# andywag/streaming_data_loader

Hardware: AMD Instinct MI355X
Metric: device-resident tokenize+mask MB/s of input text, seq_len=512, 1/2/4/8 MI355X (higher is better)
Workload: dtype u8->int32

## Files before the change

### streaming_data_loader_amd/csrc/kernels.hpp

```cpp
#pragma once

#include <hip/hip_runtime.h>

#include <cstdint>

#include "common.hpp"
#include "zstd_format.hpp"

namespace sdl {

hipError_t launch_chunk_ranges(const uint64_t *off, int64_t R, int64_t N, uint32_t *ranges, hipStream_t st,
                               uint32_t *rb1 = nullptr, uint32_t *zero1 = nullptr, const void *copy_src = nullptr,
                               void *copy_dst = nullptr, size_t copy_bytes = 0);

hipError_t launch_wordpiece_chunks(const DevTok &T, const DevFirst &F, bool cased, const uint8_t *text, int64_t N,
                                   const uint64_t *off, int64_t R,
                                   uint32_t *ranges, uint16_t *tokc, uint32_t *chunk_cnt, uint32_t *rec_local,
                                   hipStream_t st, int64_t c_begin = 0, int64_t c_end = -1);

struct BpeLong {
    uint64_t pos;
    uint32_t len;
    uint32_t chunk;
    uint32_t k;
// ... 87 lines not shown
    const uint64_t *nominal;
    const uint64_t *found;
    uint32_t n_chunks;
    const uint32_t *tgt0;
    uint16_t *slots;
    uint32_t cap;
    uint64_t *end_bit;
    uint64_t *end_hdr;
    uint32_t *next;
    uint32_t *len;
    uint32_t *flags;
    int32_t *status;
    const uint64_t *mend;
};
hipError_t launch_gz_find(const uint8_t *in, uint64_t ma, uint64_t mz, const uint64_t *nominal, uint64_t n_chunks,
                          uint64_t span, uint64_t *found, uint32_t *stats, hipStream_t st);
hipError_t launch_inflate_chunks(const uint8_t *in, const GzChunkArgs &a, uint64_t n_list, hipStream_t st);
inline uint64_t gz_window_group(uint64_t n) {
    uint64_t g = 1;
    while (g * g < n) ++g;
    return g;
}
hipError_t launch_gz_windows(const uint16_t *slots, uint32_t cap, const uint32_t *order, const uint32_t *len,
                             uint64_t n_order, uint8_t *windows, uint16_t *gmaps, uint8_t *gwin, hipStream_t st);
hipError_t launch_gz_resolve(const uint16_t *slots, uint32_t cap, const uint32_t *order, const uint32_t *len,
                             const uint64_t *pos, uint64_t n_order, const uint8_t *windows, uint8_t *out,
                             uint32_t *crc, uint32_t *shift, const X2N &x2n, int32_t *status, hipStream_t st);
hipError_t launch_gz_crc_fold(const uint32_t *crc, const uint32_t *shift, uint64_t n_order, const uint8_t *trailer,
                              const int32_t *status, int32_t *mstatus, hipStream_t st);

int64_t scan_tmp_words(int64_t n);
hipError_t launch_exclusive_scan(const uint32_t *in, uint32_t *out, int64_t n, uint32_t *tmp, hipStream_t st,
                                 const uint32_t *carry_in = nullptr);

enum : int32_t {
    ZS_OK = zs::OK,
    ZS_E_RANGE = zs::E_RANGE,
    ZS_E_TRUNC = zs::E_TRUNC,
    ZS_E_MAGIC = zs::E_MAGIC,
    ZS_E_DICT = zs::E_DICT,
    ZS_E_WINDOW = zs::E_WINDOW,
    ZS_E_BTYPE = zs::E_BTYPE,
    ZS_E_BSIZE = zs::E_BSIZE,
    ZS_E_LITHDR = zs::E_LITHDR,
    ZS_E_HUF = zs::E_HUF,
    ZS_E_FSE = zs::E_FSE,
    ZS_E_SEQHDR = zs::E_SEQHDR,
    ZS_E_ENDBITS = zs::E_ENDBITS,
    ZS_E_FAR = zs::E_FAR,
    ZS_E_SIZE = zs::E_SIZE,
    ZS_E_CHECKSUM = zs::E_CHECKSUM,
    ZS_E_STALL = zs::E_STALL
};
hipError_t launch_zs_index(const uint8_t *zst, uint64_t len, const uint64_t *foff, uint64_t n, zs::Frame *frames,
                           zs::Block *blocks, const uint32_t *first_block, uint32_t *nblk, uint32_t block_cap,
                           hipStream_t st);
hipError_t launch_zs_parse(const uint8_t *zst, const zs::Frame *frames, zs::Block *blocks, uint32_t nb, hipStream_t st);
hipError_t launch_zs_link(zs::Frame *frames, zs::Block *blocks, uint64_t n, uint32_t *lit_tot, uint32_t *seq_tot,
                          unsigned long long *totals, hipStream_t st);
hipError_t launch_zs_decode(const uint8_t *zst, const zs::Frame *frames, zs::Block *blocks, uint32_t nb,
                            const uint32_t *lit_base, const uint32_t *seq_base, uint8_t *lit, zs::SeqRec *seq,
                            hipStream_t st);
hipError_t launch_zs_chain(zs::Frame *frames, zs::Block *blocks, uint64_t n, uint32_t *out_size,
                           unsigned long long *totals, hipStream_t st);
hipError_t launch_zs_write(const uint8_t *zst, zs::Frame *frames, const zs::Block *blocks, uint32_t nb, uint64_t n,
                           const uint32_t *lit_base, const uint32_t *seq_base, const uint8_t *lit, const zs::SeqRec *seq,
                           const uint32_t *ooff, uint8_t *out, bool check, int32_t *status, uint32_t *bad,
                           hipStream_t st, hipEvent_t *ev = nullptr);

constexpr int MAX_SEGMENTS = 16;
struct SegChunks {
    int64_t cb[MAX_SEGMENTS + 1];
    int K;
};
hipError_t launch_seg_bounds(const uint32_t *ranges, const SegChunks &sc, int64_t R, uint32_t *rb, hipStream_t st);
hipError_t launch_scan_range(const uint32_t *in, uint32_t *out, const uint32_t *rb, int k, hipStream_t st);

hipError_t launch_compact_tokens(const uint32_t *tokc, const uint32_t *chunk_cnt, const uint32_t *chunk_off,
                                 int64_t n_chunks, uint32_t *tok, const uint32_t *long_count,
                                 const uint32_t *chunk_ent, const BpeLong *long_list, const uint16_t *long_scratch,
                                 hipStream_t st, const uint32_t *long_pool = nullptr, int64_t stride = STAGE,
                                 bool list16 = false);


struct SegSel {
    const uint32_t *rb;
    int k;
    int last;
};

hipError_t launch_records(const RowParams &P, const uint64_t *off, int64_t R, int64_t N, const uint32_t *chunk_off,
                          int64_t n_chunks, const uint32_t *rec_local, uint32_t *rec_tok, uint32_t *rec_cnt,
                          uint32_t *rec_rows, SegSel sel, hipStream_t st);

struct DirectDst {
    int32_t *ids[2], *am[2], *tt[2], *lab[2];
    uint32_t base, cap, B, pad;
};
struct RowOut {
    int32_t *input_ids, *attention_mask, *token_type_ids, *labels;
    float *labels_f32;
    DirectDst direct;
};

constexpr int64_t SMALL_CHUNKS = 64;
struct SmallDown {
    const uint32_t *tokc, *chunk_cnt;
    uint32_t *chunk_off, *tok;
    const uint32_t *long_count, *chunk_ent;
    const BpeLong *long_list;
    const uint16_t *long_scratch;
    const uint32_t *long_pool;
    int64_t stride;
    int list16;
    const uint32_t *rec_local;
    uint32_t *rec_tok, *rec_cnt, *rec_rows, *row_off, *row_rec;
    uint32_t *stat;
    const uint32_t *tok_err;
    int rows;
    RowOut out;
};
hipError_t launch_downstream_small(const SmallDown &d, const RowParams &P, const uint64_t *off, int64_t R, int64_t N,
                                   hipStream_t st);

struct TokSrc {
    const uint32_t *tok;
    const uint16_t *lists;
    const uint32_t *chunk_off;
    int64_t n_lists;
    const uint32_t *row_chunk;
};

struct RowChunkIn {
    uint32_t *row_chunk;
    const uint32_t *rec_tok, *rec_cnt, *chunk_off;
    const uint64_t *off;
    int64_t n_lists;
    int32_t S, n_pre, chunk;
};
hipError_t launch_row_map(const uint32_t *row_off, int64_t R, uint32_t *row_rec, SegSel sel, hipStream_t st,
                          const RowChunkIn *rc = nullptr);

struct RowSeg {
    int32_t *ids, *am, *tt, *lab;
    uint32_t g0, n, dst, pad;
};
hipError_t launch_rows_to_host(const RowSeg *segs, int n_segs, uint32_t rows_per_seg_max, const int32_t *ids,
                               const int32_t *am, const int32_t *tt, const int32_t *lab, int S, int LW,
                               hipStream_t st);

hipError_t launch_rows_direct(const DirectDst &d, const uint32_t *row_off, int64_t R, const int32_t *ids,
                              const int32_t *am, const int32_t *tt, const int32_t *lab, int S, int LW,
                              const uint32_t *err0, const uint32_t *err1, uint32_t *stat, hipStream_t st);

struct MaskPolicy {
    int32_t policy;
    int32_t per_mille;
    uint32_t vocab_size;
    uint32_t pad;
    const uint32_t *cont_bits;
};

hipError_t launch_rows(const RowParams &P, const TokSrc &src, const uint32_t *rec_tok, const uint32_t *rec_cnt,
                       const uint32_t *row_off, const uint32_t *row_rec, SegSel sel, int64_t rows_cap, RowOut out,
                       hipStream_t st,
                       hipStream_t st_late = nullptr, const MaskPolicy *mp = nullptr);
struct PackParams {
    const uint32_t *tok, *rec_tok, *rec_cnt;
    uint32_t *rec_len;
    uint32_t *pk_off;
    int64_t R, rows_cap;
    int32_t S, B, eos, min_ids;
    const int32_t *carry_ids, *carry_pos;
    const uint32_t *carry_len;
// ... 59 lines not shown
```

### streaming_data_loader_amd/csrc/pipeline.hip

```cpp
#include "common.hpp"
#include "device_util.hpp"
#include "kernels.hpp"
#include "rows_device.hpp"

namespace sdl {

constexpr int SCAN_NT = 256;
constexpr int SCAN_PER = 8;
constexpr int SCAN_TILE = SCAN_NT * SCAN_PER;

__global__ __launch_bounds__(SCAN_NT) void k_scan_reduce(const uint32_t *__restrict__ in, int64_t n,
                                                         uint32_t *__restrict__ sums) {
    __shared__ uint32_t scratch[SCAN_NT / 64];
    const int64_t base = (int64_t)blockIdx.x * SCAN_TILE + (int64_t)threadIdx.x * SCAN_PER;
    uint32_t s = 0;
#pragma unroll
    for (int k = 0; k < SCAN_PER; ++k)
        if (base + k < n) s += in[base + k];
    uint32_t tot;
    block_excl_sum<SCAN_NT>(s, &tot, scratch);
    if (threadIdx.x == 0) sums[blockIdx.x] = tot;
}

__global__ __launch_bounds__(SCAN_NT) void k_scan_sums(uint32_t *__restrict__ sums, int64_t nb,
                                                       const uint32_t *carry_in) {
    __shared__ uint32_t scratch[SCAN_NT / 64];
    uint32_t carry = carry_in ? *carry_in : 0u;
    for (int64_t t0 = 0; t0 < nb; t0 += SCAN_TILE) {
        const int64_t base = t0 + (int64_t)threadIdx.x * SCAN_PER;
        uint32_t v[SCAN_PER], s = 0;
#pragma unroll
        for (int k = 0; k < SCAN_PER; ++k) {
            v[k] = base + k < nb ? sums[base + k] : 0u;
            s += v[k];
        }
        uint32_t tot;
        uint32_t ex = block_excl_sum<SCAN_NT>(s, &tot, scratch) + carry;
#pragma unroll
        for (int k = 0; k < SCAN_PER; ++k) {
            if (base + k < nb) sums[base + k] = ex;
            ex += v[k];
        }
        carry += tot;
    }
    if (threadIdx.x == 0) sums[nb] = carry;
}

__global__ __launch_bounds__(SCAN_NT) void k_scan_apply(const uint32_t *__restrict__ in, int64_t n,
                                                        const uint32_t *__restrict__ sums, int64_t nb,
                                                        uint32_t *__restrict__ out) {
    __shared__ uint32_t scratch[SCAN_NT / 64];
    const int64_t base = (int64_t)blockIdx.x * SCAN_TILE + (int64_t)threadIdx.x * SCAN_PER;
    uint32_t v[SCAN_PER], s = 0;
#pragma unroll
    for (int k = 0; k < SCAN_PER; ++k) {
        v[k] = base + k < n ? in[base + k] : 0u;
        s += v[k];
    }
    uint32_t tot;
    uint32_t ex = block_excl_sum<SCAN_NT>(s, &tot, scratch) + sums[blockIdx.x];
#pragma unroll
    for (int k = 0; k < SCAN_PER; ++k) {
        if (base + k < n) out[base + k] = ex;
        ex += v[k];
    }
    if (blockIdx.x == 0 && threadIdx.x == 0) out[n] = sums[nb];
}

constexpr int SCAN_SMALL_NT = 1024, SCAN_SMALL_PER = 8;
constexpr int64_t SCAN_SMALL = (int64_t)SCAN_SMALL_NT * SCAN_SMALL_PER;
__global__ __launch_bounds__(SCAN_SMALL_NT) void k_scan_small(const uint32_t *__restrict__ in, int64_t n,
                                                              uint32_t *__restrict__ out, const uint32_t *carry_in) {
    __shared__ uint32_t scratch[SCAN_SMALL_NT / 64];
    const uint32_t carry = carry_in ? *carry_in : 0u;
    __syncthreads();
    const int64_t base = (int64_t)threadIdx.x * SCAN_SMALL_PER;
    uint32_t v[SCAN_SMALL_PER], s = 0;
#pragma unroll
    for (int k = 0; k < SCAN_SMALL_PER; ++k) {
        v[k] = base + k < n ? in[base + k] : 0u;
        s += v[k];
    }
    uint32_t tot;
    uint32_t ex = block_excl_sum<SCAN_SMALL_NT>(s, &tot, scratch) + carry;
#pragma unroll
    for (int k = 0; k < SCAN_SMALL_PER; ++k) {
        if (base + k < n) out[base + k] = ex;
        ex += v[k];
    }
    if (threadIdx.x == 0) out[n] = carry + tot;
}

int64_t scan_tmp_words(int64_t n) { return (n + SCAN_TILE - 1) / SCAN_TILE + 1; }

hipError_t launch_exclusive_scan(const uint32_t *in, uint32_t *out, int64_t n, uint32_t *tmp, hipStream_t st,
                                 const uint32_t *carry_in) {
    if (n <= 0) return carry_in ? hipSuccess : hipMemsetAsync(out, 0, sizeof(uint32_t), st);
    if (n <= SCAN_SMALL) {
        hipLaunchKernelGGL(k_scan_small, dim3(1), dim3(SCAN_SMALL_NT), 0, st, in, n, out, carry_in);
        return hipGetLastError();
    }
    const int64_t nb = (n + SCAN_TILE - 1) / SCAN_TILE;
    hipLaunchKernelGGL(k_scan_reduce, dim3((unsigned)nb), dim3(SCAN_NT), 0, st, in, n, tmp);
    hipLaunchKernelGGL(k_scan_sums, dim3(1), dim3(SCAN_NT), 0, st, tmp, nb, carry_in);
    hipLaunchKernelGGL(k_scan_apply, dim3((unsigned)nb), dim3(SCAN_NT), 0, st, in, n, tmp, nb, out);
    return hipGetLastError();
}

__global__ void k_seg_bounds(const uint32_t *__restrict__ ranges, SegChunks sc, int64_t R, uint32_t *__restrict__ rb) {
    const int k = (int)threadIdx.x;
    if (k > sc.K) return;
    uint32_t v;
    if (k == 0) v = 0;
    else if (k == sc.K) v = (uint32_t)R;
    else {
        const uint32_t q = ranges[3 * sc.cb[k] + 2];
        v = q == 0 ? 0u : q - 1u;
        if (v > (uint32_t)R) v = (uint32_t)R;
    }
    rb[k] = v;
}

hipError_t launch_seg_bounds(const uint32_t *ranges, const SegChunks &sc, int64_t R, uint32_t *rb, hipStream_t st) {
    hipLaunchKernelGGL(k_seg_bounds, dim3(1), dim3(64), 0, st, ranges, sc, R, rb);
    return hipGetLastError();
}

constexpr int RSCAN_NT = 1024, RSCAN_PER = 8;
__global__ __launch_bounds__(RSCAN_NT) void k_scan_range(const uint32_t *__restrict__ in, uint32_t *__restrict__ out,
                                                         const uint32_t *__restrict__ rb, int k) {
    __shared__ uint32_t scratch[RSCAN_NT / 64];
    const int64_t a = rb[k], b = rb[k + 1];
    uint32_t carry = k > 0 ? out[a] : 0u;
    __syncthreads();
    for (int64_t t0 = a; t0 < b; t0 += (int64_t)RSCAN_NT * RSCAN_PER) {
        const int64_t base = t0 + (int64_t)threadIdx.x * RSCAN_PER;
        uint32_t v[RSCAN_PER], sum = 0;
#pragma unroll
        for (int j = 0; j < RSCAN_PER; ++j) {
            v[j] = base + j < b ? in[base + j] : 0u;
// ... 3 lines not shown
        uint32_t ex = block_excl_sum<RSCAN_NT>(sum, &tot, scratch) + carry;
#pragma unroll
        for (int j = 0; j < RSCAN_PER; ++j) {
            if (base + j < b) out[base + j] = ex;
            ex += v[j];
        }
        carry += tot;
    }
    if (threadIdx.x == 0) out[b] = carry;
}

hipError_t launch_scan_range(const uint32_t *in, uint32_t *out, const uint32_t *rb, int k, hipStream_t st) {
    hipLaunchKernelGGL(k_scan_range, dim3(1), dim3(RSCAN_NT), 0, st, in, out, rb, k);
    return hipGetLastError();
}

struct RowSpan {
    int64_t g_lo, g_real, g_end;
};
__device__ __forceinline__ RowSpan row_span(const SegSel &s, const uint32_t *row_off, int B, int64_t rows_cap) {
    const uint32_t r0 = s.rb[s.k], r1 = s.rb[s.k + 1];
    RowSpan x;
    x.g_lo = row_off[r0];
    x.g_real = row_off[r1];
    x.g_end = x.g_real;
    if (s.last) {
        int64_t Gpad = (x.g_real + B - 1) / B * B;
        if (Gpad > rows_cap) Gpad = rows_cap;
        x.g_end = Gpad > x.g_real ? Gpad : x.g_real;
    }
    return x;
}

__global__ __launch_bounds__(256) void k_chunk_ranges(const uint64_t *__restrict__ off, int64_t R, int64_t n_chunks,
                                                      uint32_t *__restrict__ ranges, uint32_t *__restrict__ rb1,
                                                      uint32_t *__restrict__ zero1, const uint4 *__restrict__ csrc,
                                                      uint4 *__restrict__ cdst, int64_t cn16) {
    const int64_t c = (int64_t)blockIdx.x * 256 + threadIdx.x;
    for (int64_t x = c; x < cn16; x += (int64_t)gridDim.x * 256) cdst[x] = csrc[x];
    if (c == 0) {
        if (rb1) {
            rb1[0] = 0u;
            rb1[1] = (uint32_t)R;
        }
        if (zero1) *zero1 = 0u;
    }
    if (c >= n_chunks) return;
    auto lower = [&](int64_t x) {
        int64_t lo = 0, hi = R + 1;
        while (lo < hi) {
            const int64_t m = (lo + hi) >> 1;
            if ((int64_t)off[m] < x) lo = m + 1; else hi = m;
        }
        return lo;
    };
    const int64_t c0 = c * CHUNK;
    ranges[3 * c + 0] = (uint32_t)lower(c0 - HALO_L);
    ranges[3 * c + 1] = (uint32_t)lower(c0 - HALO_L + WIN);
    ranges[3 * c + 2] = (uint32_t)lower(c0);
}

hipError_t launch_chunk_ranges(const uint64_t *off, int64_t R, int64_t N, uint32_t *ranges, hipStream_t st,
                               uint32_t *rb1, uint32_t *zero1, const void *copy_src, void *copy_dst, size_t copy_bytes) {
    const int64_t n_chunks = (N + CHUNK - 1) / CHUNK;
    const int64_t cn16 = copy_src ? (int64_t)((copy_bytes + 15) / 16) : 0;
    if (n_chunks == 0 && cn16 == 0) return hipSuccess;
    int64_t blocks = (n_chunks + 255) / 256;
    const int64_t cb = (cn16 + 255) / 256;
    if (cb > blocks) blocks = cb < 64 ? cb : 64;
    if (blocks < 1) blocks = 1;
    hipLaunchKernelGGL(k_chunk_ranges, dim3((unsigned)blocks), dim3(256), 0, st, off, R, n_chunks, ranges, rb1, zero1,
                       (const uint4 *)copy_src, (uint4 *)copy_dst, cn16);
    return hipGetLastError();
}

template <int PART, bool E16 = false>
__global__ __launch_bounds__(256) void k_compact_tokens(const uint32_t *__restrict__ tokc,
                                                        const uint32_t *__restrict__ chunk_cnt,
                                                        const uint32_t *__restrict__ chunk_off, int64_t n_chunks,
                                                        uint32_t *__restrict__ tok, const uint32_t *long_count,
                                                        const uint32_t *__restrict__ chunk_ent,
                                                        const BpeLong *__restrict__ long_list,
// ... 4 lines not shown
    compact_wave<PART, E16>(cb, tokc, chunk_cnt, chunk_off, n_chunks, tok, long_count, chunk_ent, long_list,
                            long_scratch, long_pool, stride);
}

hipError_t launch_compact_tokens(const uint32_t *tokc, const uint32_t *chunk_cnt, const uint32_t *chunk_off,
                                 int64_t n_chunks, uint32_t *tok, const uint32_t *long_count,
                                 const uint32_t *chunk_ent, const BpeLong *long_list, const uint16_t *long_scratch,
                                 hipStream_t st, const uint32_t *long_pool, int64_t stride, bool list16) {
    if (n_chunks == 0) return hipSuccess;
    const int64_t waves = (n_chunks + COMPACT_CPW - 1) / COMPACT_CPW;
    if (list16) {
        hipLaunchKernelGGL((k_compact_tokens<1, true>), dim3((unsigned)((waves + 3) / 4)), dim3(256), 0, st, tokc,
                           chunk_cnt, chunk_off, n_chunks, tok, nullptr, nullptr, nullptr, nullptr, nullptr, stride);
        return hipGetLastError();
    }
    hipLaunchKernelGGL(k_compact_tokens<1>, dim3((unsigned)((waves + 3) / 4)), dim3(256), 0, st, tokc, chunk_cnt,
                       chunk_off, n_chunks, tok, long_count, chunk_ent, long_list, long_scratch, long_pool, stride);
    if (long_count)
        hipLaunchKernelGGL(k_compact_tokens<2>, dim3((unsigned)((waves + 3) / 4)), dim3(256), 0, st, tokc, chunk_cnt,
                           chunk_off, n_chunks, tok, long_count, chunk_ent, long_list, long_scratch, long_pool, stride);
    return hipGetLastError();
}

__global__ __launch_bounds__(256) void k_records(RowParams P, const uint64_t *__restrict__ off, int64_t R, int64_t N,
                                                 const uint32_t *__restrict__ chunk_off, int64_t n_chunks,
                                                 const uint32_t *__restrict__ rec_local, uint32_t *__restrict__ rec_tok,
                                                 uint32_t *__restrict__ rec_cnt, uint32_t *__restrict__ rec_rows,
                                                 SegSel sel) {
    const int64_t r_lo = sel.rb[sel.k], r_hi = sel.rb[sel.k + 1];
    for (int64_t r = r_lo + (int64_t)blockIdx.x * 256 + threadIdx.x; r < r_hi; r += (int64_t)gridDim.x * 256)
        record_one(P, off, r, N, chunk_off, n_chunks, rec_local, rec_tok, rec_cnt, rec_rows);
}

hipError_t launch_records(const RowParams &P, const uint64_t *off, int64_t R, int64_t N, const uint32_t *chunk_off,
                          int64_t n_chunks, const uint32_t *rec_local, uint32_t *rec_tok, uint32_t *rec_cnt,
                          uint32_t *rec_rows, SegSel sel, hipStream_t st) {
    if (R == 0) return hipSuccess;
    const int64_t want = (R + 255) / 256;
    hipLaunchKernelGGL(k_records, dim3((unsigned)(want < 1024 ? want : 1024)), dim3(256), 0, st, P, off, R, N,
                       chunk_off, n_chunks, rec_local, rec_tok, rec_cnt, rec_rows, sel);
    return hipGetLastError();
}

template <bool RC>
__global__ __launch_bounds__(256) void k_row_map(const uint32_t *__restrict__ row_off, uint32_t *__restrict__ row_rec,
                                                 SegSel sel, RowChunkIn rc) {
    const int64_t r_lo = sel.rb[sel.k], r_hi = sel.rb[sel.k + 1];
    for (int64_t r = r_lo + (int64_t)blockIdx.x * 256 + threadIdx.x; r < r_hi; r += (int64_t)gridDim.x * 256) {
        const uint32_t g0 = row_off[r], g1 = row_off[r + 1];
        if constexpr (RC) {
            if (g0 == g1) continue;
            ListBracket br = list_bracket(rc.off[r], rc.off[r + 1], rc.n_lists);
            const uint32_t t0 = rc.rec_tok[r], cnt = rc.rec_cnt[r];
            for (uint32_t g = g0; g < g1; ++g) {
                row_rec[g] = (uint32_t)r;
                const int64_t base = rc.chunk ? (int64_t)(g - g0) * rc.S : 0;
                const int64_t rel0 = base > rc.n_pre ? base - rc.n_pre : 0;
                if (rel0 < (int64_t)cnt) br.lo = list_chunk_of(rc.chunk_off, br.lo, br.hi, t0 + (uint32_t)rel0);
                rc.row_chunk[g] = (uint32_t)br.lo;
            }
        } else {
            for (uint32_t g = g0; g < g1; ++g) row_rec[g] = (uint32_t)r;
        }
    }
}

__device__ __forceinline__ void block_scan_small(const uint32_t *__restrict__ in, int64_t n, uint32_t *__restrict__ out,
                                                 uint32_t *scratch) {
    const int64_t base = (int64_t)threadIdx.x * SCAN_SMALL_PER;
    uint32_t v[SCAN_SMALL_PER], s = 0;
#pragma unroll
    for (int k = 0; k < SCAN_SMALL_PER; ++k) {
        v[k] = base + k < n ? in[base + k] : 0u;
        s += v[k];
    }
    uint32_t tot;
    uint32_t ex = block_excl_sum<SCAN_SMALL_NT>(s, &tot, scratch);
#pragma unroll
    for (int k = 0; k < SCAN_SMALL_PER; ++k) {
        if (base + k < n) out[base + k] = ex;
        ex += v[k];
    }
    if (threadIdx.x == 0) out[n] = tot;
}

hipError_t launch_row_map(const uint32_t *row_off, int64_t R, uint32_t *row_rec, SegSel sel, hipStream_t st,
                          const RowChunkIn *rc) {
    if (R == 0) return hipSuccess;
    const int64_t want = (R + 255) / 256;
    const dim3 grid((unsigned)(want < 1024 ? want : 1024));
    if (rc) hipLaunchKernelGGL(k_row_map<true>, grid, dim3(256), 0, st, row_off, row_rec, sel, *rc);
    else hipLaunchKernelGGL(k_row_map<false>, grid, dim3(256), 0, st, row_off, row_rec, sel, RowChunkIn{});
    return hipGetLastError();
}

constexpr int ROWS_WAVES = 7;
constexpr int ROWS_WAVES4 = 1;
// ... 1301 lines not shown
```

### streaming_data_loader_amd/csrc/rows_device.hpp

```cpp
#pragma once
#include "common.hpp"
#include "device_util.hpp"
#include "kernels.hpp"
#include "list_index.hpp"
#include "mlm_pick.hpp"

namespace sdl {

static_assert(LIST_CHUNK == CHUNK && LIST_STRIDE == STAGE, "list_index.hpp restates the chunk geometry");

constexpr int COMPACT_CPW = 4;
template <int PART = 0, bool E16 = false>
__device__ __forceinline__ void compact_wave(int64_t cb, const uint32_t *__restrict__ tokc,
                                             const uint32_t *__restrict__ chunk_cnt,
                                             const uint32_t *__restrict__ chunk_off, int64_t n_chunks,
                                             uint32_t *__restrict__ tok, const uint32_t *long_count,
                                             const uint32_t *__restrict__ chunk_ent,
                                             const BpeLong *__restrict__ long_list,
                                             const uint16_t *__restrict__ long_scratch,
                                             const uint32_t *__restrict__ long_pool, int64_t stride) {
    const int lane = threadIdx.x & 63;
    uint32_t n[COMPACT_CPW], o[COMPACT_CPW];
#pragma unroll
    for (int j = 0; j < COMPACT_CPW; ++j) {
// ... 75 lines not shown
                    const uint16_t *jr = reinterpret_cast<const uint16_t *>(tokc + (cb + j) * stride + UNI_JR_OFF) +
                                         (x[j] & 0xFFFu);
                    for (uint32_t q0 = 0; q0 < w[j]; q0 += 8) {
                        uint32_t id[8];
#pragma unroll
                        for (uint32_t r = 0; r < 8; ++r) id[r] = q0 + r < w[j] ? jr[q0 + r] : 0u;
#pragma unroll
                        for (uint32_t r = 0; r < 8; ++r)
                            if (q0 + r < w[j]) dst[at + q0 + r] = id[r];
                    }
                } else if (long_pool) {
                    const uint32_t po = x[j] & 0x7FFFFFFFu;
                    for (uint32_t q = 0; q < w[j]; ++q) dst[at + q] = long_pool[po + 1 + q];
                } else {
                    const uint64_t pos = long_list[x[j] & 0x7FFFFFFFu].pos;
                    for (uint32_t q = 0; q < w[j]; ++q) dst[at + q] = long_scratch[pos + q];
                }
            }
            written[j] += (uint32_t)lane_bcast((int)incl, 63);
        }
    }
}

__device__ __forceinline__ void compact_small(const SmallDown &d, int64_t cb, const uint32_t *__restrict__ chunk_off,
                                              int64_t n_chunks) {
    if (d.list16)
        compact_wave<0, true>(cb, d.tokc, d.chunk_cnt, chunk_off, n_chunks, d.tok, nullptr, nullptr, nullptr, nullptr,
                              nullptr, d.stride);
    else
        compact_wave(cb, d.tokc, d.chunk_cnt, chunk_off, n_chunks, d.tok, d.long_count, d.chunk_ent, d.long_list,
                     d.long_scratch, d.long_pool, d.stride);
}

__device__ __forceinline__ void record_one(const RowParams &P, const uint64_t *__restrict__ off, int64_t r, int64_t N,
                                           const uint32_t *__restrict__ chunk_off, int64_t n_chunks,
                                           const uint32_t *__restrict__ rec_local, uint32_t *__restrict__ rec_tok,
                                           uint32_t *__restrict__ rec_cnt, uint32_t *__restrict__ rec_rows) {
    auto tok_off = [&](int64_t q) -> uint32_t {
        const int64_t p = (int64_t)off[q];
        return p >= N ? chunk_off[n_chunks] : chunk_off[p / CHUNK] + rec_local[q];
    };
    const uint32_t a = tok_off(r), b = tok_off(r + 1);
    const uint32_t cnt = b - a;
    const uint32_t n = cnt + (uint32_t)(P.n_pre + P.n_post);
    uint32_t rows = 0;
    if (n >= (uint32_t)P.min_ids) rows = P.chunk ? ceil_div_u32(n, (uint32_t)P.S) : 1u;
    rec_tok[r] = a;
    rec_cnt[r] = cnt;
    rec_rows[r] = rows;
}

__device__ __forceinline__ uint4 philox4x32_10(uint4 c, uint32_t k0, uint32_t k1) {
#pragma unroll
    for (int r = 0; r < 10; ++r) {
        const uint32_t lo0 = 0xD2511F53u * c.x, hi0 = __umulhi(0xD2511F53u, c.x);
        const uint32_t lo1 = 0xCD9E8D57u * c.z, hi1 = __umulhi(0xCD9E8D57u, c.z);
        c = make_uint4(hi1 ^ c.y ^ k0, lo1, hi0 ^ c.w ^ k1, lo0);
        k0 += 0x9E3779B9u;
        k1 += 0xBB67AE85u;
    }
    return c;
}

__device__ __forceinline__ uint32_t mlm_key(uint64_t seed, uint64_t rec, uint32_t chunk, uint32_t pos) {
    const uint4 c = philox4x32_10(make_uint4(pos >> 2, chunk, (uint32_t)rec, (uint32_t)(rec >> 32)), (uint32_t)seed,
                                  (uint32_t)(seed >> 32));
    const uint32_t s = pos & 3u;
    return s == 0 ? c.x : s == 1 ? c.y : s == 2 ? c.z : c.w;
}

__device__ __forceinline__ int32_t frame_id(const int32_t (&a)[MAX_FRAME], int k) {
    return k == 0 ? a[0] : k == 1 ? a[1] : k == 2 ? a[2] : a[3];
}

template <int MR>
__device__ __forceinline__ void select_k_smallest(const uint32_t (&key)[MR][4], int k, bool (&sel)[MR][4]) {
    if (k <= 0) {
#pragma unroll
        for (int m = 0; m < MR; ++m)
#pragma unroll
            for (int w = 0; w < 4; ++w) sel[m][w] = false;
        return;
// ... 595 lines not shown
```

### streaming_data_loader_amd/csrc/sdl_batcher.cpp

```cpp
#include <dlfcn.h>
#include <hip/hip_runtime.h>

#include <algorithm>
#include <chrono>
#include <cstdlib>
#include <cmath>
#include <cstdio>
#include <cstring>
#include <deque>
#include <memory>
#include <mutex>
#include <stdexcept>
#include <string>
#include <thread>
#include <vector>

#include "../../include/sdl_batcher.h"
#include "assets.hpp"
#include "kernels.hpp"
#include "pack_queue.hpp"

using namespace sdl;

namespace {
// ... 433 lines not shown
        HIP_TRY(launch_pack_flush(pack_params(0, rows_cap), st));
        pk_cur ^= 1;
        pk_ran = true;
        last_rows_cap = rows_cap;
        last_R = 0;
    }

    int64_t rows_capacity(int64_t N, int64_t R) const {
        const int64_t F = P.n_pre + P.n_post;
        const int64_t ids = dt.kind == TOK_UNIGRAM ? 2 * N + 1024 * 1024 : N;
        int64_t cap = P.chunk ? (ids + R * (F + P.S - 1)) / P.S + 1 : R;
        if (pack()) cap = (ids + R + P.S - 1) / P.S + 1;
        return (cap + P.B - 1) / P.B * P.B;
    }

    void run_device(const uint8_t *d_text, int64_t N, const uint64_t *d_off, int64_t R, uint64_t first_record,
                    hipStream_t st, const uint32_t *d_labels = nullptr, const uint64_t *d_label_off = nullptr) {
        const int64_t n_chunks = (N + CHUNK - 1) / CHUNK;
        const int64_t rows_cap = rows_capacity(N, R);
        if (pack() && rows_cap * P.S > ((int64_t)1 << 32) - 4096)
            throw CapacityError("pack: the call's rows exceed 2^32 positions");
        ranges.ensure((size_t)std::max<int64_t>(n_chunks, 1) * 3);
        const bool wp = dt.kind != TOK_BYTE_BPE && dt.kind != TOK_UNIGRAM;
        tokc.ensure((size_t)std::max<int64_t>(n_chunks, 1) * (dt.kind == TOK_UNIGRAM ? UNI_STAGE : wp ? STAGE / 2 : STAGE));
        chunk_cnt.ensure((size_t)n_chunks + 1);
        chunk_off.ensure((size_t)n_chunks + 1);
        rec_local.ensure((size_t)R + 1);
        const size_t tok_ids_n = dt.kind == TOK_UNIGRAM ? (size_t)2 * N + 1024 * 1024 + 1 : (size_t)N + 1;
        if (!wp || span()) tok_ids.ensure(tok_ids_n);
        rec_tok.ensure((size_t)R + 1);
        rec_cnt.ensure((size_t)R + 1);
        rec_rows.ensure((size_t)R + 1);
        row_off.ensure((size_t)R + 1);
        scan_tmp.ensure((size_t)std::max(scan_tmp_words(n_chunks), scan_tmp_words(R)) + 1);
        const size_t plane = (size_t)std::max<int64_t>(rows_cap, 1) * P.S;
        o_ids.ensure(plane);
        o_am.ensure(plane);
        if (plane4()) o_tt.ensure(plane);
        if (multi()) {
            o_f32.ensure((size_t)std::max<int64_t>(rows_cap, 1) * P.label_width);
            lab_err.ensure(1);
        } else {
            o_lab.ensure((size_t)std::max<int64_t>(rows_cap, 1) * P.label_width);
            if (single()) lab_err.ensure(1);
        }
        row_rec.ensure((size_t)std::max<int64_t>(rows_cap, 1));
        const bool rm1 = P.task == SDL_TASK_MLM && P.rng_mode == 1;
        const bool policy = P.task == SDL_TASK_MLM && mpol.policy != 0;
        const int mask_w = (P.S + 31) / 32;

        RowParams p = P;
        p.first_record = first_record;
        p.mask_w = mask_w;
        p.mask_bits0 = nullptr;
        p.mask_spos = nullptr;
        p.mask_off = d_off;
        p.mask_R = R;
        p.mask_spec1 = 0;
        const bool bpe = dt.kind == TOK_BYTE_BPE;
        const bool uni = dt.kind == TOK_UNIGRAM;
        SegChunks sc{};
        sc.K = 1;
        if (!bpe && !uni && seg_target > 1 && n_chunks >= 2 * seg_min_chunks) {
            sc.K = (int)std::min<int64_t>(seg_target, n_chunks / seg_min_chunks);
            sc.K = std::min(sc.K, MAX_SEGMENTS);
        }
        for (int k = 0; k <= sc.K; ++k) sc.cb[k] = n_chunks * k / sc.K;
// ... 45 lines not shown
            SmallDown d{tokc.p, chunk_cnt.p, chunk_off.p, tok_ids.p,
                        uni ? uni_counters.p : bpe ? long_count.p : nullptr,
                        uni || bpe ? chunk_ent.p : nullptr, bpe ? long_list.p : nullptr,
                        bpe ? long_scratch.p : nullptr, uni ? uni_pool.p : nullptr,
                        uni ? (int64_t)UNI_STAGE : (int64_t)STAGE, wp ? 1 : 0, rec_local.p, rec_tok.p, rec_cnt.p,
                        rec_rows.p, row_off.p, row_rec.p, fused_done ? fuse_stat : nullptr,
                        uni ? uni_err.p : nullptr, 0, out};
            d.rows = fused_done && !rm1 && !policy ? 1 : 0;
            return d;
        };
        auto downstream = [&](int k, hipStream_t s) {
            const SegSel sel{seg_rb.p, k, k == sc.K - 1 ? 1 : 0};
            const int64_t ca = sc.cb[k], cz = sc.cb[k + 1];
            bool rows_done = false;
            if (small) {
                const SmallDown d = small_down();
                rows_done = d.rows != 0;
                HIP_TRY(launch_downstream_small(d, p, d_off, R, N, s));
            } else {
            if (!piped) mark(2);
            HIP_TRY(launch_exclusive_scan(chunk_cnt.p + ca, chunk_off.p + ca, cz - ca, scan_tmp.p, s,
                                          k > 0 ? chunk_off.p + ca : nullptr));
            if (!piped) mark(3);
            if (uni)
                HIP_TRY(launch_compact_tokens(tokc.p, chunk_cnt.p, chunk_off.p, n_chunks, tok_ids.p, uni_counters.p,
                                              chunk_ent.p, nullptr, nullptr, s, uni_pool.p, UNI_STAGE));
            else if (bpe)
                HIP_TRY(launch_compact_tokens(tokc.p, chunk_cnt.p, chunk_off.p, n_chunks, tok_ids.p, long_count.p,
                                              chunk_ent.p, long_list.p, long_scratch.p, s));
            else if (!from_lists)
                HIP_TRY(launch_compact_tokens(tokc.p + ca * (STAGE / 2), chunk_cnt.p + ca, chunk_off.p + ca, cz - ca,
                                              tok_ids.p, nullptr, nullptr, nullptr, nullptr, s, nullptr, STAGE, true));
            if (!piped) mark(4);
            HIP_TRY(launch_records(p, d_off, R, N, chunk_off.p, n_chunks, rec_local.p, rec_tok.p, rec_cnt.p, rec_rows.p,
                                   sel, s));
            if (!piped) mark(5);
            if (pack()) {
                mark(6);
                run_pack(R, rows_cap, s);
                return;
            }
            if (piped) HIP_TRY(launch_scan_range(rec_rows.p, row_off.p, seg_rb.p, k, s));
            else HIP_TRY(launch_exclusive_scan(rec_rows.p, row_off.p, R, scan_tmp.p, s));
            const RowChunkIn rc{row_chunk.p, rec_tok.p, rec_cnt.p, chunk_off.p, d_off, cz, P.S, P.n_pre, P.chunk};
            HIP_TRY(launch_row_map(row_off.p, R, row_rec.p, sel, s, from_lists ? &rc : nullptr));
            }
            const TokSrc src = from_lists ? TokSrc{nullptr, lists, chunk_off.p, cz, row_chunk.p}
                                          : TokSrc{tok_ids.p, nullptr, nullptr, 0, nullptr};
            if (!piped) mark(6);
            if (span()) {
                span_err.ensure(1);
                SpanPlan pl{};
                const bool two_phase = span_two_phase;
                if (two_phase) {
                    pl.capr = P.label_width / 2 + 2;
                    span_tab.ensure((size_t)std::max<int64_t>(rows_cap, 1) * (size_t)pl.capr);
                    span_meta.ensure((size_t)std::max<int64_t>(rows_cap, 1));
                    span_ovf.ensure((size_t)std::max<int64_t>(rows_cap, 1) + 1);
                    pl.tab = span_tab.p;
                    pl.meta = span_meta.p;
                    pl.ovf_n = span_ovf.p;
                    pl.ovf_list = span_ovf.p + 1;
                }
                HIP_TRY(launch_rows_span(p, tok_ids.p, rec_tok.p, rec_cnt.p, row_off.p, row_rec.p, sel, rows_cap, out,
                                         span_err.p, s, two_phase ? &pl : nullptr));
            } else {
                if (rm1 && rec0) {
                    HIP_TRY(hipStreamWaitEvent(s, rand_ev[1], 0));
                    HIP_TRY(launch_rows(p, src, rec_tok.p, rec_cnt.p, row_off.p, row_rec.p, sel, rows_cap, out, s));
                } else if (!rows_done) {
                    HIP_TRY(launch_rows(p, src, rec_tok.p, rec_cnt.p, row_off.p, row_rec.p, sel, rows_cap, out, s,
                                        nullptr, policy ? &mpol : nullptr));
                }
            }
            if (multi())
                HIP_TRY(launch_multi_labels(d_labels, d_label_off, row_rec.p, row_off.p, sel, rows_cap, P.B,
                                            P.label_width, o_f32.p, lab_err.p, s));
            else if (single())
// ... 2010 lines not shown
```

Measured before the change: 237,000.

## Fuse record tile sums with row scan and map; cut scan kernel launches

The large exclusive scan drops from three kernels to two: the reduce kernel also writes the carry, and each apply block recomputes its prefix from the tile sums, with at most 1024 blocks. The records kernel can now emit per-tile row sums, so the row-offset scan and the row map run in one fused kernel, removing a separate scan and map launch in the non-piped path. Chunk-range lookup stages a bracket of record offsets in shared memory after a wave-parallel search, so the per-thread binary searches hit LDS instead of global memory. In exchange there is redundant prefix summation per block and extra shared-memory use.

```diff
diff --git a/streaming_data_loader_amd/csrc/kernels.hpp b/streaming_data_loader_amd/csrc/kernels.hpp
--- a/streaming_data_loader_amd/csrc/kernels.hpp
+++ b/streaming_data_loader_amd/csrc/kernels.hpp
@@ -143,6 +143,7 @@
 int64_t scan_tmp_words(int64_t n);
 hipError_t launch_exclusive_scan(const uint32_t *in, uint32_t *out, int64_t n, uint32_t *tmp, hipStream_t st,
                                  const uint32_t *carry_in = nullptr);
+int64_t scan_small_max();
 
 enum : int32_t {
     ZS_OK = zs::OK,
@@ -200,9 +201,10 @@
     int last;
 };
 
+int64_t records_tile_words(int64_t R);
 hipError_t launch_records(const RowParams &P, const uint64_t *off, int64_t R, int64_t N, const uint32_t *chunk_off,
                           int64_t n_chunks, const uint32_t *rec_local, uint32_t *rec_tok, uint32_t *rec_cnt,
-                          uint32_t *rec_rows, SegSel sel, hipStream_t st);
+                          uint32_t *rec_rows, SegSel sel, hipStream_t st, uint32_t *tile_sums = nullptr);
 
 struct DirectDst {
     int32_t *ids[2], *am[2], *tt[2], *lab[2];
@@ -251,6 +253,8 @@
 };
 hipError_t launch_row_map(const uint32_t *row_off, int64_t R, uint32_t *row_rec, SegSel sel, hipStream_t st,
                           const RowChunkIn *rc = nullptr);
+hipError_t launch_scan_rows_map(const uint32_t *rec_rows, int64_t R, const uint32_t *tile_sums, uint32_t *row_off,
+                                uint32_t *row_rec, hipStream_t st, const RowChunkIn *rc = nullptr);
 
 struct RowSeg {
     int32_t *ids, *am, *tt, *lab;
diff --git a/streaming_data_loader_amd/csrc/pipeline.hip b/streaming_data_loader_amd/csrc/pipeline.hip
--- a/streaming_data_loader_amd/csrc/pipeline.hip
+++ b/streaming_data_loader_amd/csrc/pipeline.hip
@@ -8,9 +8,11 @@
 constexpr int SCAN_NT = 256;
 constexpr int SCAN_PER = 8;
 constexpr int SCAN_TILE = SCAN_NT * SCAN_PER;
+constexpr int64_t SCAN_MAX_BLOCKS = 1024;
 
 __global__ __launch_bounds__(SCAN_NT) void k_scan_reduce(const uint32_t *__restrict__ in, int64_t n,
-                                                         uint32_t *__restrict__ sums) {
+                                                         uint32_t *__restrict__ sums, int64_t nb,
+                                                         const uint32_t *carry_in) {
     __shared__ uint32_t scratch[SCAN_NT / 64];
     const int64_t base = (int64_t)blockIdx.x * SCAN_TILE + (int64_t)threadIdx.x * SCAN_PER;
     uint32_t s = 0;
@@ -19,52 +21,44 @@
         if (base + k < n) s += in[base + k];
     uint32_t tot;
     block_excl_sum<SCAN_NT>(s, &tot, scratch);
-    if (threadIdx.x == 0) sums[blockIdx.x] = tot;
-}
-
-__global__ __launch_bounds__(SCAN_NT) void k_scan_sums(uint32_t *__restrict__ sums, int64_t nb,
-                                                       const uint32_t *carry_in) {
+    if (threadIdx.x == 0) {
+        sums[blockIdx.x] = tot;
+        if (blockIdx.x == 0) sums[nb] = carry_in ? *carry_in : 0u;
+    }
+}
+
+__device__ __forceinline__ uint32_t block_sum_before(const uint32_t *__restrict__ sums, int64_t t_lo,
+                                                     uint32_t *scratch) {
+    uint32_t p = 0, tot;
+    for (int64_t i = threadIdx.x; i < t_lo; i += SCAN_NT) p += sums[i];
+    block_excl_sum<SCAN_NT>(p, &tot, scratch);
+    return tot;
+}
+
+__global__ __launch_bounds__(SCAN_NT) void k_scan_apply(const uint32_t *__restrict__ in, int64_t n,
+                                                        const uint32_t *__restrict__ sums, int64_t nb, int64_t tpb,
+                                                        uint32_t *__restrict__ out) {
     __shared__ uint32_t scratch[SCAN_NT / 64];
-    uint32_t carry = carry_in ? *carry_in : 0u;
-    for (int64_t t0 = 0; t0 < nb; t0 += SCAN_TILE) {
-        const int64_t base = t0 + (int64_t)threadIdx.x * SCAN_PER;
+    const int64_t t_lo = (int64_t)blockIdx.x * tpb, t_hi = t_lo + tpb < nb ? t_lo + tpb : nb;
+    uint32_t carry = block_sum_before(sums, t_lo, scratch) + sums[nb];
+    for (int64_t t = t_lo; t < t_hi; ++t) {
+        const int64_t base = t * SCAN_TILE + (int64_t)threadIdx.x * SCAN_PER;
         uint32_t v[SCAN_PER], s = 0;
 #pragma unroll
         for (int k = 0; k < SCAN_PER; ++k) {
-            v[k] = base + k < nb ? sums[base + k] : 0u;
+            v[k] = base + k < n ? in[base + k] : 0u;
             s += v[k];
         }
         uint32_t tot;
         uint32_t ex = block_excl_sum<SCAN_NT>(s, &tot, scratch) + carry;
 #pragma unroll
         for (int k = 0; k < SCAN_PER; ++k) {
-            if (base + k < nb) sums[base + k] = ex;
+            if (base + k < n) out[base + k] = ex;
             ex += v[k];
         }
         carry += tot;
     }
-    if (threadIdx.x == 0) sums[nb] = carry;
-}
-
-__global__ __launch_bounds__(SCAN_NT) void k_scan_apply(const uint32_t *__restrict__ in, int64_t n,
-                                                        const uint32_t *__restrict__ sums, int64_t nb,
-                                                        uint32_t *__restrict__ out) {
-    __shared__ uint32_t scratch[SCAN_NT / 64];
-    const int64_t base = (int64_t)blockIdx.x * SCAN_TILE + (int64_t)threadIdx.x * SCAN_PER;
-    uint32_t v[SCAN_PER], s = 0;
-#pragma unroll
-    for (int k = 0; k < SCAN_PER; ++k) {
-        v[k] = base + k < n ? in[base + k] : 0u;
-        s += v[k];
-    }
-    uint32_t tot;
-    uint32_t ex = block_excl_sum<SCAN_NT>(s, &tot, scratch) + sums[blockIdx.x];
-#pragma unroll
-    for (int k = 0; k < SCAN_PER; ++k) {
-        if (base + k < n) out[base + k] = ex;
-        ex += v[k];
-    }
-    if (blockIdx.x == 0 && threadIdx.x == 0) out[n] = sums[nb];
+    if (t_hi == nb && threadIdx.x == 0) out[n] = carry;
 }
 
 constexpr int SCAN_SMALL_NT = 1024, SCAN_SMALL_PER = 8;
@@ -101,11 +95,14 @@
         return hipGetLastError();
     }
     const int64_t nb = (n + SCAN_TILE - 1) / SCAN_TILE;
-    hipLaunchKernelGGL(k_scan_reduce, dim3((unsigned)nb), dim3(SCAN_NT), 0, st, in, n, tmp);
-    hipLaunchKernelGGL(k_scan_sums, dim3(1), dim3(SCAN_NT), 0, st, tmp, nb, carry_in);
-    hipLaunchKernelGGL(k_scan_apply, dim3((unsigned)nb), dim3(SCAN_NT), 0, st, in, n, tmp, nb, out);
+    const int64_t tpb = (nb + SCAN_MAX_BLOCKS - 1) / SCAN_MAX_BLOCKS;
+    hipLaunchKernelGGL(k_scan_reduce, dim3((unsigned)nb), dim3(SCAN_NT), 0, st, in, n, tmp, nb, carry_in);
+    hipLaunchKernelGGL(k_scan_apply, dim3((unsigned)((nb + tpb - 1) / tpb)), dim3(SCAN_NT), 0, st, in, n, tmp, nb, tpb,
+                       out);
     return hipGetLastError();
 }
+
+int64_t scan_small_max() { return SCAN_SMALL; }
 
 __global__ void k_seg_bounds(const uint32_t *__restrict__ ranges, SegChunks sc, int64_t R, uint32_t *__restrict__ rb) {
     const int k = (int)threadIdx.x;
@@ -175,10 +172,13 @@
     return x;
 }
 
+constexpr int RANGES_CAP = 2048;
 __global__ __launch_bounds__(256) void k_chunk_ranges(const uint64_t *__restrict__ off, int64_t R, int64_t n_chunks,
                                                       uint32_t *__restrict__ ranges, uint32_t *__restrict__ rb1,
                                                       uint32_t *__restrict__ zero1, const uint4 *__restrict__ csrc,
                                                       uint4 *__restrict__ cdst, int64_t cn16) {
+    __shared__ uint64_t s_off[RANGES_CAP];
+    __shared__ int64_t s_br[2];
     const int64_t c = (int64_t)blockIdx.x * 256 + threadIdx.x;
     for (int64_t x = c; x < cn16; x += (int64_t)gridDim.x * 256) cdst[x] = csrc[x];
     if (c == 0) {
@@ -188,9 +188,47 @@
         }
         if (zero1) *zero1 = 0u;
     }
+    const int64_t cA = (int64_t)blockIdx.x * 256;
+    if (cA >= n_chunks) return;
+    const int64_t cZ = cA + 255 < n_chunks ? cA + 255 : n_chunks - 1;
+    const int64_t xa = cA * CHUNK - HALO_L, xz = cZ * CHUNK - HALO_L + WIN;
+    const int wid = (int)(threadIdx.x >> 6), lane = lane_id();
+    if (wid < 2) {
+        const int64_t x = wid == 0 ? xa : xz;
+        int64_t lo = 0, hi = R + 1;
+        while (lo < hi) {
+            const int64_t st = (hi - lo + 63) >> 6, m = lo + lane * st;
+            const bool below = m < hi && (int64_t)off[m] < x;
+            const int cnt = __popcll(__ballot(below));
+            if (cnt == 0) {
+                hi = lo;
+            } else {
+                const int64_t h = lo + cnt * st;
+                lo = lo + (cnt - 1) * st + 1;
+                hi = h < hi ? h : hi;
+            }
+        }
+        if (lane == 0) s_br[wid] = lo;
+    }
+    __syncthreads();
+    const int64_t b_lo = s_br[0], b_hi = s_br[1];
+    const bool fits = b_hi - b_lo <= RANGES_CAP;
+    if (fits) {
+        for (int64_t i = threadIdx.x; i < b_hi - b_lo; i += 256) s_off[i] = off[b_lo + i];
+        __syncthreads();
+    }
     if (c >= n_chunks) return;
     auto lower = [&](int64_t x) {
         int64_t lo = 0, hi = R + 1;
+        if (fits) {
+            lo = b_lo;
+            hi = b_hi;
+            while (lo < hi) {
+                const int64_t m = (lo + hi) >> 1;
+                if ((int64_t)s_off[m - b_lo] < x) lo = m + 1; else hi = m;
+            }
+            return lo;
+        }
         while (lo < hi) {
             const int64_t m = (lo + hi) >> 1;
             if ((int64_t)off[m] < x) lo = m + 1; else hi = m;
@@ -261,37 +299,105 @@
         record_one(P, off, r, N, chunk_off, n_chunks, rec_local, rec_tok, rec_cnt, rec_rows);
 }
 
+constexpr int REC_TILE = 256;
+__global__ __launch_bounds__(REC_TILE) void k_records_tiles(RowParams P, const uint64_t *__restrict__ off, int64_t R,
+                                                            int64_t N, const uint32_t *__restrict__ chunk_off,
+                                                            int64_t n_chunks, const uint32_t *__restrict__ rec_local,
+                                                            uint32_t *__restrict__ rec_tok,
+                                                            uint32_t *__restrict__ rec_cnt,
+                                                            uint32_t *__restrict__ rec_rows,
+                                                            uint32_t *__restrict__ tile_sums) {
+    __shared__ uint32_t scratch[REC_TILE / 64];
+    const int64_t nt = (R + REC_TILE - 1) / REC_TILE;
+    for (int64_t t = blockIdx.x; t < nt; t += gridDim.x) {
+        const int64_t r = t * REC_TILE + threadIdx.x;
+        uint32_t rows = 0, tot;
+        if (r < R) rows = record_one(P, off, r, N, chunk_off, n_chunks, rec_local, rec_tok, rec_cnt, rec_rows);
+        block_excl_sum<REC_TILE>(rows, &tot, scratch);
+        if (threadIdx.x == 0) tile_sums[t] = tot;
+    }
+}
+
+int64_t records_tile_words(int64_t R) { return (R + REC_TILE - 1) / REC_TILE + 1; }
+
 hipError_t launch_records(const RowParams &P, const uint64_t *off, int64_t R, int64_t N, const uint32_t *chunk_off,
                           int64_t n_chunks, const uint32_t *rec_local, uint32_t *rec_tok, uint32_t *rec_cnt,
-                          uint32_t *rec_rows, SegSel sel, hipStream_t st) {
+                          uint32_t *rec_rows, SegSel sel, hipStream_t st, uint32_t *tile_sums) {
     if (R == 0) return hipSuccess;
     const int64_t want = (R + 255) / 256;
-    hipLaunchKernelGGL(k_records, dim3((unsigned)(want < 1024 ? want : 1024)), dim3(256), 0, st, P, off, R, N,
-                       chunk_off, n_chunks, rec_local, rec_tok, rec_cnt, rec_rows, sel);
+    const dim3 grid((unsigned)(want < 1024 ? want : 1024));
+    if (tile_sums)
+        hipLaunchKernelGGL(k_records_tiles, grid, dim3(REC_TILE), 0, st, P, off, R, N, chunk_off, n_chunks, rec_local,
+                           rec_tok, rec_cnt, rec_rows, tile_sums);
+    else
+        hipLaunchKernelGGL(k_records, grid, dim3(256), 0, st, P, off, R, N, chunk_off, n_chunks, rec_local, rec_tok,
+                           rec_cnt, rec_rows, sel);
     return hipGetLastError();
+}
+
+template <bool RC>
+__device__ __forceinline__ void row_map_one(int64_t r, uint32_t g0, uint32_t g1, uint32_t *__restrict__ row_rec,
+                                            const RowChunkIn &rc) {
+    if constexpr (RC) {
+        if (g0 == g1) return;
+        ListBracket br = list_bracket(rc.off[r], rc.off[r + 1], rc.n_lists);
+        const uint32_t t0 = rc.rec_tok[r], cnt = rc.rec_cnt[r];
+        for (uint32_t g = g0; g < g1; ++g) {
+            row_rec[g] = (uint32_t)r;
+            const int64_t base = rc.chunk ? (int64_t)(g - g0) * rc.S : 0;
+            const int64_t rel0 = base > rc.n_pre ? base - rc.n_pre : 0;
+            if (rel0 < (int64_t)cnt) br.lo = list_chunk_of(rc.chunk_off, br.lo, br.hi, t0 + (uint32_t)rel0);
+            rc.row_chunk[g] = (uint32_t)br.lo;
+        }
+    } else {
+        for (uint32_t g = g0; g < g1; ++g) row_rec[g] = (uint32_t)r;
+    }
 }
 
 template <bool RC>
 __global__ __launch_bounds__(256) void k_row_map(const uint32_t *__restrict__ row_off, uint32_t *__restrict__ row_rec,
                                                  SegSel sel, RowChunkIn rc) {
     const int64_t r_lo = sel.rb[sel.k], r_hi = sel.rb[sel.k + 1];
-    for (int64_t r = r_lo + (int64_t)blockIdx.x * 256 + threadIdx.x; r < r_hi; r += (int64_t)gridDim.x * 256) {
-        const uint32_t g0 = row_off[r], g1 = row_off[r + 1];
-        if constexpr (RC) {
-            if (g0 == g1) continue;
-            ListBracket br = list_bracket(rc.off[r], rc.off[r + 1], rc.n_lists);
-            const uint32_t t0 = rc.rec_tok[r], cnt = rc.rec_cnt[r];
-            for (uint32_t g = g0; g < g1; ++g) {
-                row_rec[g] = (uint32_t)r;
-                const int64_t base = rc.chunk ? (int64_t)(g - g0) * rc.S : 0;
-                const int64_t rel0 = base > rc.n_pre ? base - rc.n_pre : 0;
-                if (rel0 < (int64_t)cnt) br.lo = list_chunk_of(rc.chunk_off, br.lo, br.hi, t0 + (uint32_t)rel0);
-                rc.row_chunk[g] = (uint32_t)br.lo;
-            }
-        } else {
-            for (uint32_t g = g0; g < g1; ++g) row_rec[g] = (uint32_t)r;
-        }
-    }
+    for (int64_t r = r_lo + (int64_t)blockIdx.x * 256 + threadIdx.x; r < r_hi; r += (int64_t)gridDim.x * 256)
+        row_map_one<RC>(r, row_off[r], row_off[r + 1], row_rec, rc);
+}
+
+template <bool RC>
+__global__ __launch_bounds__(REC_TILE) void k_scan_rows_map(const uint32_t *__restrict__ rec_rows, int64_t R,
+                                                            const uint32_t *__restrict__ tile_sums, int64_t nt,
+                                                            int64_t tpb, uint32_t *__restrict__ row_off,
+                                                            uint32_t *__restrict__ row_rec, RowChunkIn rc) {
+    static_assert(REC_TILE == SCAN_NT, "block_sum_before strides by SCAN_NT");
+    __shared__ uint32_t scratch[REC_TILE / 64];
+    const int64_t t_lo = (int64_t)blockIdx.x * tpb, t_hi = t_lo + tpb < nt ? t_lo + tpb : nt;
+    uint32_t carry = block_sum_before(tile_sums, t_lo, scratch);
+    for (int64_t t = t_lo; t < t_hi; ++t) {
+        const int64_t r = t * REC_TILE + threadIdx.x;
+        const uint32_t v = r < R ? rec_rows[r] : 0u;
+        uint32_t tot;
+        const uint32_t g0 = block_excl_sum<REC_TILE>(v, &tot, scratch) + carry;
+        if (r < R) {
+            row_off[r] = g0;
+            row_map_one<RC>(r, g0, g0 + v, row_rec, rc);
+        }
+        carry += tot;
+    }
+    if (t_hi == nt && threadIdx.x == 0) row_off[R] = carry;
+}
+
+hipError_t launch_scan_rows_map(const uint32_t *rec_rows, int64_t R, const uint32_t *tile_sums, uint32_t *row_off,
+                                uint32_t *row_rec, hipStream_t st, const RowChunkIn *rc) {
+    if (R <= 0) return hipErrorInvalidValue;
+    const int64_t nt = (R + REC_TILE - 1) / REC_TILE;
+    const int64_t tpb = (nt + SCAN_MAX_BLOCKS - 1) / SCAN_MAX_BLOCKS;
+    const dim3 grid((unsigned)((nt + tpb - 1) / tpb));
+    if (rc)
+        hipLaunchKernelGGL(k_scan_rows_map<true>, grid, dim3(REC_TILE), 0, st, rec_rows, R, tile_sums, nt, tpb, row_off,
+                           row_rec, *rc);
+    else
+        hipLaunchKernelGGL(k_scan_rows_map<false>, grid, dim3(REC_TILE), 0, st, rec_rows, R, tile_sums, nt, tpb,
+                           row_off, row_rec, RowChunkIn{});
+    return hipGetLastError();
 }
 
 __device__ __forceinline__ void block_scan_small(const uint32_t *__restrict__ in, int64_t n, uint32_t *__restrict__ out,
diff --git a/streaming_data_loader_amd/csrc/rows_device.hpp b/streaming_data_loader_amd/csrc/rows_device.hpp
--- a/streaming_data_loader_amd/csrc/rows_device.hpp
+++ b/streaming_data_loader_amd/csrc/rows_device.hpp
@@ -131,10 +131,10 @@
                      d.long_scratch, d.long_pool, d.stride);
 }
 
-__device__ __forceinline__ void record_one(const RowParams &P, const uint64_t *__restrict__ off, int64_t r, int64_t N,
-                                           const uint32_t *__restrict__ chunk_off, int64_t n_chunks,
-                                           const uint32_t *__restrict__ rec_local, uint32_t *__restrict__ rec_tok,
-                                           uint32_t *__restrict__ rec_cnt, uint32_t *__restrict__ rec_rows) {
+__device__ __forceinline__ uint32_t record_one(const RowParams &P, const uint64_t *__restrict__ off, int64_t r, int64_t N,
+                                               const uint32_t *__restrict__ chunk_off, int64_t n_chunks,
+                                               const uint32_t *__restrict__ rec_local, uint32_t *__restrict__ rec_tok,
+                                               uint32_t *__restrict__ rec_cnt, uint32_t *__restrict__ rec_rows) {
     auto tok_off = [&](int64_t q) -> uint32_t {
         const int64_t p = (int64_t)off[q];
         return p >= N ? chunk_off[n_chunks] : chunk_off[p / CHUNK] + rec_local[q];
@@ -147,6 +147,7 @@
     rec_tok[r] = a;
     rec_cnt[r] = cnt;
     rec_rows[r] = rows;
+    return rows;
 }
 
 __device__ __forceinline__ uint4 philox4x32_10(uint4 c, uint32_t k0, uint32_t k1) {
diff --git a/streaming_data_loader_amd/csrc/sdl_batcher.cpp b/streaming_data_loader_amd/csrc/sdl_batcher.cpp
--- a/streaming_data_loader_amd/csrc/sdl_batcher.cpp
+++ b/streaming_data_loader_amd/csrc/sdl_batcher.cpp
@@ -489,7 +489,7 @@
         rec_cnt.ensure((size_t)R + 1);
         rec_rows.ensure((size_t)R + 1);
         row_off.ensure((size_t)R + 1);
-        scan_tmp.ensure((size_t)std::max(scan_tmp_words(n_chunks), scan_tmp_words(R)) + 1);
+        scan_tmp.ensure((size_t)std::max({scan_tmp_words(n_chunks), scan_tmp_words(R), records_tile_words(R)}) + 1);
         const size_t plane = (size_t)std::max<int64_t>(rows_cap, 1) * P.S;
         o_ids.ensure(plane);
         o_am.ensure(plane);
@@ -601,18 +601,24 @@
                 HIP_TRY(launch_compact_tokens(tokc.p + ca * (STAGE / 2), chunk_cnt.p + ca, chunk_off.p + ca, cz - ca,
                                               tok_ids.p, nullptr, nullptr, nullptr, nullptr, s, nullptr, STAGE, true));
             if (!piped) mark(4);
+            const bool scan_map = !piped && !pack() && R > scan_small_max();
             HIP_TRY(launch_records(p, d_off, R, N, chunk_off.p, n_chunks, rec_local.p, rec_tok.p, rec_cnt.p, rec_rows.p,
-                                   sel, s));
+                                   sel, s, scan_map ? scan_tmp.p : nullptr));
             if (!piped) mark(5);
             if (pack()) {
                 mark(6);
                 run_pack(R, rows_cap, s);
                 return;
             }
-            if (piped) HIP_TRY(launch_scan_range(rec_rows.p, row_off.p, seg_rb.p, k, s));
-            else HIP_TRY(launch_exclusive_scan(rec_rows.p, row_off.p, R, scan_tmp.p, s));
             const RowChunkIn rc{row_chunk.p, rec_tok.p, rec_cnt.p, chunk_off.p, d_off, cz, P.S, P.n_pre, P.chunk};
-            HIP_TRY(launch_row_map(row_off.p, R, row_rec.p, sel, s, from_lists ? &rc : nullptr));
+            if (scan_map) {
+                HIP_TRY(launch_scan_rows_map(rec_rows.p, R, scan_tmp.p, row_off.p, row_rec.p, s,
+                                             from_lists ? &rc : nullptr));
+            } else {
+                if (piped) HIP_TRY(launch_scan_range(rec_rows.p, row_off.p, seg_rb.p, k, s));
+                else HIP_TRY(launch_exclusive_scan(rec_rows.p, row_off.p, R, scan_tmp.p, s));
+                HIP_TRY(launch_row_map(row_off.p, R, row_rec.p, sel, s, from_lists ? &rc : nullptr));
+            }
             }
             const TokSrc src = from_lists ? TokSrc{nullptr, lists, chunk_off.p, cz, row_chunk.p}
                                           : TokSrc{tok_ids.p, nullptr, nullptr, 0, nullptr};
```

Result: faster. 241,600 (median of 6 runs) (+1.9%).
